# JuliaRobotics/IncrementalInference.jl

Hardware: AMD Instinct MI355X
Metric: clique-messages/sec (higher is better)
Workload: dtype f64; 1 GPU; config 2: ContinuousEuclid(2) 1000-variable odometry chain + priors every 100, N=200 particles, nested-dissection order, full up+down solveTree; variables_per_gpu=1000, particles=200, cliques=983, parallelism=single GPU

## Files before the change

### include/nbp.h

```cpp
#ifndef NBP_H
#define NBP_H

#include <stdint.h>

#ifdef __cplusplus
extern "C" {
#endif

#define NBP_MAXV 6
#define NBP_MAXF 128
#define NBP_MAXD 3
#define NBP_MAXC 4
#define NBP_MAXK 8
#define NBP_MAXN 512
#define NBP_COMP_STRIDE 13
enum nbp_dist {
  NBP_DIST_GAUSSIAN = 0,
  NBP_DIST_UNIFORM = 1,
  NBP_DIST_RAYLEIGH = 2,
  NBP_DIST_TABLE = 3
};

typedef int32_t nbp_status;
#define NBP_OK 0
// ... 65 lines not shown
typedef struct nbp_diag {
  int64_t solves;
  int64_t nonconverged;
  int64_t nan_results;
  int64_t residual_evals;
  int64_t lcv_evals;
  int64_t lcv_evals_f32;
  int64_t proposal_launches_workgroup;
  int64_t proposal_launches_wave;
  int64_t proposal_launches_split;
  int64_t lane_side_launches;
  int64_t lane_waits;
  int64_t lane_side_updates;
  int64_t sunk_updates;
  int64_t sink_launches;
} nbp_diag;

typedef struct nbp_ctx nbp_ctx;

int64_t nbp_arena_bytes(int32_t N, int32_t n_slots);
int64_t nbp_slot_stride_doubles(int32_t N);
nbp_status nbp_ctx_create(int32_t device, int32_t N, int32_t n_slots, void *arena,
                          int64_t arena_bytes, int32_t side_ints, nbp_ctx **out);
nbp_status nbp_ctx_destroy(nbp_ctx *ctx);
nbp_status nbp_ctx_attach(nbp_ctx *ctx, void *obj, void (*destroy)(void *obj));
void *nbp_ctx_attached(const nbp_ctx *ctx);
const char *nbp_last_error(void);
nbp_status nbp_synchronize(nbp_ctx *ctx);
void *nbp_arena_ptr(nbp_ctx *ctx);
void *nbp_stream_ptr(nbp_ctx *ctx);
// ... 278 lines not shown
nbp_status nbp_program_finalize(nbp_program *prog);
nbp_status nbp_program_run(nbp_program *prog, int32_t first_stage, int32_t last_stage );
nbp_status nbp_program_reseed(nbp_program *prog, uint64_t salt);
nbp_status nbp_program_num_seeds(nbp_program *prog, int32_t *out);
nbp_status nbp_program_set_seeds(nbp_program *prog, const uint64_t *seeds, int32_t n);
nbp_status nbp_program_seed_order(nbp_program *prog, int32_t *order, int32_t n);
nbp_status nbp_program_num_stages(nbp_program *prog, int32_t *out);
nbp_status nbp_program_num_fused(nbp_program *prog, int32_t *out);
nbp_status nbp_program_num_two_stream(nbp_program *prog, int32_t *out);
nbp_status nbp_program_set_lanes(nbp_program *prog, int32_t stage, const int32_t *lane_of_descriptor, int32_t n);
typedef struct nbp_lane_part_rec {
  int32_t stage, lane, first_desc, n, wait, signals;
} nbp_lane_part_rec;
nbp_status nbp_program_lane_plan(nbp_program *prog, nbp_lane_part_rec *out, int32_t cap, int32_t *n_out);
nbp_status nbp_program_sink_plan(nbp_program *prog, int32_t *gained, int32_t cap, int32_t *n_out);
nbp_status nbp_program_destroy(nbp_program *prog);
nbp_status nbp_program_retire(nbp_program *prog);

#define NBP_COMM_ID_BYTES 128
typedef struct nbp_comm nbp_comm;
#ifndef NBP_XFER_DEFINED
#define NBP_XFER_DEFINED
typedef struct nbp_xfer { int32_t peer; int32_t slot; } nbp_xfer;
#endif
nbp_status nbp_comm_unique_id(void *id_out );
nbp_status nbp_comm_create(nbp_ctx *ctx, int32_t world, int32_t rank, const void *id, nbp_comm **out);
nbp_status nbp_comm_destroy(nbp_comm *comm);
nbp_status nbp_comm_info(nbp_comm *comm, int32_t *nranks_out, int32_t *rank_out);
nbp_status nbp_exchange(nbp_ctx *ctx, nbp_comm *comm, const nbp_xfer *sends, int32_t n_sends, const nbp_xfer *recvs, int32_t n_recvs);

// ... 68 lines not shown
```

### incrementalinference.jl_amd/abi.py

```python
import ctypes as C
import os

MAXV, MAXF, MAXD, MAXC, MAXN, COMP_STRIDE = 6, 128, 3, 4, 512, 13

EUCLID1, EUCLID2, EUCLID3, CIRCULAR, SE2 = 1, 2, 3, 4, 5
F_PRIOR, F_MSGPRIOR, F_LINREL, F_CIRCULAR, F_SE2, F_EUCLIDDIST, F_PASSTHROUGH = 1, 2, 3, 4, 5, 6, 7
DIST_GAUSSIAN, DIST_UNIFORM, DIST_RAYLEIGH, DIST_TABLE = 0, 1, 2, 3
STAGE_PROPOSALS, STAGE_PRODUCTS, STAGE_COPIES, STAGE_DECONV, STAGE_COPY_POINTS = 1, 2, 3, 4, 5
OPT_LAZY_BANDWIDTH = 1
OPT_GRAPH_REPLAY = 2
OPT_FUSED_UPDATES = 3
OPT_ASYNC_UPLOAD = 4
OPT_UP_PASS_SINKS = 5

MANIFOLD_DIM = {EUCLID1: 1, EUCLID2: 2, EUCLID3: 3, CIRCULAR: 1, SE2: 3}
MANIFOLD_P = {EUCLID1: 1, EUCLID2: 2, EUCLID3: 3, CIRCULAR: 1, SE2: 6}


class ProposalDesc(C.Structure):
    _fields_ = [
        ("factor_kind", C.c_int32),
        ("manifold", C.c_int32),
        ("nvars", C.c_int32),
        ("sfidx", C.c_int32),
# ... 152 lines not shown
    _fields_ = [
        ("solves", C.c_int64),
        ("nonconverged", C.c_int64),
        ("nan_results", C.c_int64),
        ("residual_evals", C.c_int64),
        ("lcv_evals", C.c_int64),
        ("lcv_evals_f32", C.c_int64),
        ("proposal_launches_workgroup", C.c_int64),
        ("proposal_launches_wave", C.c_int64),
        ("proposal_launches_split", C.c_int64),
        ("lane_side_launches", C.c_int64),
        ("lane_waits", C.c_int64),
        ("lane_side_updates", C.c_int64),
        ("sunk_updates", C.c_int64),
        ("sink_launches", C.c_int64),
    ]


class LanePartRec(C.Structure):
    _fields_ = [("stage", C.c_int32), ("lane", C.c_int32), ("first_desc", C.c_int32), ("n", C.c_int32), ("wait", C.c_int32), ("signals", C.c_int32)]


class ProductPlanReq(C.Structure):
    _fields_ = [(k, C.c_int32) for k in ("N", "n", "F", "D", "mani", "geom_n")]


PLAN_REFUSED_BIG_IN_ROUND, PLAN_REFUSED_LDS, PLAN_REFUSED_NO_KERNEL = 1, 2, 3


class _PlanRec(C.Structure):
    def as_dict(self):
        return {k: (getattr(self, k).decode() if k == "kernel" else getattr(self, k)) for k, _ in self._fields_ if not k.startswith("pad")}


class ProductPlanRec(_PlanRec):
# ... 46 lines not shown
def slot_stride(N):
    return 3 * N + 8


_PKG_DIR = os.path.dirname(os.path.abspath(__file__))
LIB_PATH = os.path.join(_PKG_DIR, "csrc", "libnbp.so")

EXPORTS = [
    "nbp_arena_bytes", "nbp_slot_stride_doubles", "nbp_ctx_create", "nbp_ctx_destroy",
    "nbp_last_error", "nbp_synchronize", "nbp_arena_ptr", "nbp_stream_ptr", "nbp_ctx_particles", "nbp_ctx_slots", "nbp_ctx_device",
    "nbp_ctx_reserve_resident", "nbp_ctx_resident", "nbp_belief_write_batch_async", "nbp_belief_read_batch_begin", "nbp_belief_read_batch_end",
    "nbp_run_copies_async", "nbp_program_retire",
    "nbp_slot_write", "nbp_slot_read", "nbp_belief_write", "nbp_belief_read", "nbp_belief_write_batch", "nbp_belief_read_batch", "nbp_run_resample", "nbp_side_write", "nbp_side_read",
    "nbp_run_proposals", "nbp_run_bandwidth", "nbp_run_ppe", "nbp_kde_ppe", "nbp_run_evaluate", "nbp_kde_evaluate", "nbp_run_marginal_grid", "nbp_kde_marginal_grid", "nbp_run_evaluate_marginal", "nbp_run_mmd", "nbp_kde_mmd", "nbp_run_meancov", "nbp_kde_meancov", "nbp_run_kld", "nbp_kde_kld", "nbp_run_overlap", "nbp_kde_overlap", "nbp_run_overlap_search", "nbp_run_scene_grid", "nbp_run_credible", "nbp_kde_credible", "nbp_run_modes", "nbp_kde_modes", "nbp_run_mixture", "nbp_kde_mixture", "nbp_run_factor_likelihood", "nbp_factor_likelihood", "nbp_run_factor_mode_likelihood", "nbp_factor_mode_likelihood", "nbp_run_product_grid", "nbp_product_grid", "nbp_heatmap_create", "nbp_heatmap_build", "nbp_heatmap_draw", "nbp_heatmap_info", "nbp_heatmap_destroy", "nbp_heatmap_scan_eval", "nbp_heatmap_search_eval", "nbp_run_products", "nbp_run_copies", "nbp_run_deconv", "nbp_kde_bandwidth", "nbp_conv", "nbp_manifold_product",
    "nbp_program_create", "nbp_program_add_stage", "nbp_program_set_option", "nbp_program_finalize", "nbp_program_run",
    "nbp_program_reseed", "nbp_program_num_seeds", "nbp_program_set_seeds", "nbp_program_seed_order", "nbp_ctx_attach", "nbp_ctx_attached", "nbp_program_num_stages", "nbp_program_num_fused", "nbp_program_num_two_stream", "nbp_program_set_lanes", "nbp_program_lane_plan", "nbp_program_sink_plan", "nbp_program_destroy",
    "nbp_timing_enable", "nbp_timing_read", "nbp_timing_read_n", "nbp_diag_read",
    "nbp_plan_products", "nbp_plan_fits", "nbp_plan_proposals", "nbp_last_plans",
    "nbp_comm_unique_id", "nbp_comm_create", "nbp_comm_destroy", "nbp_comm_info", "nbp_exchange", "nbp_math_eval",
]

_lib = None


def load_library(path=None):
    global _lib
    if _lib is not None and path is None:
        return _lib
    path = path or os.environ.get("NBP_LIB_OVERRIDE") or LIB_PATH
    if not os.path.exists(path):
        raise RuntimeError(
# ... 92 lines not shown
    lib.nbp_program_destroy.argtypes = [vp]
    lib.nbp_comm_unique_id.argtypes = [vp]
    lib.nbp_comm_create.argtypes = [vp, i32, i32, vp, C.POINTER(vp)]
    lib.nbp_comm_destroy.argtypes = [vp]
    lib.nbp_comm_info.argtypes = [vp, ip, ip]
    lib.nbp_math_eval.argtypes = [vp, i32, dp, dp, dp, dp, i64]
    lib.nbp_exchange.argtypes = [vp, vp, C.POINTER(Xfer), i32, C.POINTER(Xfer), i32]
    lib.nbp_timing_enable.argtypes = [vp, i32]
    lib.nbp_timing_read.argtypes = [vp, dp, C.POINTER(i64)]
    lib.nbp_timing_read_n.argtypes = [vp, dp, C.POINTER(i64), i32]
    lib.nbp_program_num_fused.argtypes = [vp, C.POINTER(i32)]
    lib.nbp_program_num_two_stream.argtypes = [vp, C.POINTER(i32)]
    lib.nbp_program_set_lanes.argtypes = [vp, i32, ip, i32]
    lib.nbp_program_lane_plan.argtypes = [vp, C.POINTER(LanePartRec), i32, C.POINTER(i32)]
    lib.nbp_program_sink_plan.argtypes = [vp, C.POINTER(i32), i32, C.POINTER(i32)]
    lib.nbp_diag_read.argtypes = [vp, C.POINTER(Diag), i32]
    lib.nbp_plan_products.argtypes = [C.POINTER(ProductPlanReq), C.POINTER(ProductPlanRec), i64]
    lib.nbp_plan_fits.argtypes = [C.POINTER(FitPlanReq), C.POINTER(FitPlanRec), i64]
    lib.nbp_plan_proposals.argtypes = [C.POINTER(ProposalPlanReq), C.POINTER(ProposalPlanRec), i64]
    lib.nbp_last_plans.argtypes = [vp, C.POINTER(ProductPlanRec), C.POINTER(FitPlanRec), C.POINTER(FitPlanRec)]
    for name in EXPORTS:
        fn = getattr(lib, name)
        if fn.restype is C.c_int:
            fn.restype = C.c_int32
    if path == LIB_PATH:
        _lib = lib
    return lib
```

### incrementalinference.jl_amd/backend.py

```python
import ctypes as C
import weakref

import numpy as np

from . import abi


class NbpError(RuntimeError):
    """Hard error from libnbp (status < 0).  The Julia shim maps this to `error()`, which fails
    the clique Task and makes `monitorCSMs` tear the solve down with a CompositeException
    (reference: CliqStateMachineUtils.jl:184-246, test/testCSMMonitor.jl:51)."""


_IP, _DP = C.POINTER(C.c_int32), C.POINTER(C.c_double)


def _i32(seq):
    a = np.ascontiguousarray(seq, dtype=np.int32)
    return a, a.ctypes.data_as(_IP)


def _f64(a, shape=None):
    a = np.ascontiguousarray(a, dtype=np.float64)
    a = a if shape is None else a.reshape(shape)
# ... 712 lines not shown

    def lane_plan(self):
        n = C.c_int32(0)
        self.backend._check(self.backend.lib.nbp_program_lane_plan(self._p, None, 0, C.byref(n)))
        recs = (abi.LanePartRec * max(n.value, 1))()
        self.backend._check(self.backend.lib.nbp_program_lane_plan(self._p, recs, n.value, C.byref(n)))
        return [{k: getattr(r, k) for k, _ in abi.LanePartRec._fields_} for r in recs[:n.value]]

    def sink_plan(self):
        n = C.c_int32(0)
        self.backend._check(self.backend.lib.nbp_program_sink_plan(self._p, None, 0, C.byref(n)))
        arr = (C.c_int32 * max(n.value, 1))()
        self.backend._check(self.backend.lib.nbp_program_sink_plan(self._p, arr, n.value, C.byref(n)))
        return list(arr[:n.value])

    def num_fused(self):
        n = C.c_int32(0)
        self.backend._check(self.backend.lib.nbp_program_num_fused(self._p, C.byref(n)))
        return n.value

    def num_two_stream(self):
        n = C.c_int32(0)
        self.backend._check(self.backend.lib.nbp_program_num_two_stream(self._p, C.byref(n)))
        return n.value

    def run(self, first=0, last=-1):
        self.backend._check(self.backend.lib.nbp_program_run(self._p, first, last))

    def reseed(self, salt):
        self.backend._check(self.backend.lib.nbp_program_reseed(self._p, C.c_uint64(salt)))
# ... 40 lines not shown
```

### incrementalinference.jl_amd/csrc/nbp_api.hip

```cpp
#include <hip/hip_runtime.h>

#include <cmath>
#include <cstdio>
#include <cstring>
#include <string>
#include <thread>
#include <vector>

#include <unordered_map>

#include <dlfcn.h>
#include <algorithm>
#include <rccl/rccl.h>

#ifndef NBP_TU
#define NBP_TU 0
#endif
#include "nbp_kernels.h"
#include "nbp_fused.h"
#include "nbp_ppe.h"
#include "nbp_query.h"
#include "nbp_stats.h"
#include "nbp_marginal.h"
#include "nbp_heatmap.h"
#include "nbp_modes.h"
#include "nbp_likelihood.h"
#include "nbp_overlap.h"
#include "nbp_credible.h"
#include "nbp_mixture.h"
#include "nbp_scene.h"
#include "nbp_productgrid.h"
#include "../../include/nbp_lanes.h"
#include "../../include/nbp_sinks.h"

static thread_local std::string g_err;
static nbp_status fail(nbp_status code, const std::string &msg) {
  g_err = msg;
  return code;
}
template <class F>
static void host_parallel_for(int n, int grain, F &&f) {
  const unsigned hw = std::thread::hardware_concurrency();
  int nt = n / grain;
  if (nt > 8) nt = 8;
  if (hw && nt > (int)hw) nt = (int)hw;
  if (nt <= 1) {
    for (int i = 0; i < n; i++) f(i);
    return;
// ... 65 lines not shown
  int prop_split_min = -1;
  int64_t prop_launches[3] = {0, 0, 0};
  int fused_p1_min = 2048;
  hipStream_t stream2 = nullptr;
  hipEvent_t pipe_ev[2] = {nullptr, nullptr};
  int pipe_min = 1 << 30;
  bool no_lanes = false;
  std::vector<hipEvent_t> lane_ev;
  hipEvent_t lane_fork = nullptr, lane_join = nullptr;
  double *gstats1 = nullptr;
  size_t gstats1_doubles = 0;
  int64_t lane_side_launches = 0, lane_waits = 0, lane_side_updates = 0;
  bool no_sinks = false;
  int sink_placement = 0;
  int64_t sunk_updates = 0, sink_launches = 0;
  int lcv_p2_min = 256, lcv_p1_min = 4 * 256;
  bool fit_w5 = true, debug_occupancy = false;
  int prod_hl2_min = 192, prod_nch = 0, prod_all_levels_hl = 8;
  bool prod_xs = true, prod_lat_uni = true;
  nbp_product_plan_rec last_product{};
  nbp_fit_plan_rec last_prep{}, last_fit{};
  bool timing = false;
  std::vector<std::pair<hipEvent_t, hipEvent_t>> ev[5];
  double ms[5] = {0, 0, 0, 0, 0};
  int64_t nl[5] = {0, 0, 0, 0, 0};
};

typedef void (*nbp_product_fn)(const nbp_product_desc *, double *, const double *, int, double *, int, int64_t, int32_t *, nbp_levels);
struct nbp_product_kernel_row { nbp_product_fn fn; int HL, mani; bool xs, w1; const char *name; int lb; };
#define NBP_ROW(NAME, HL_, MANI_, XS_, W1_, LB_) {NAME, HL_, MANI_, XS_, W1_, #NAME, LB_}
// ... 141 lines not shown
  c->S = nbp_slot_stride_doubles(N);
  c->Npad = ((N + 63) / 64) * 64;
  c->P = 1024 / c->Npad;
  if (c->P > 4) c->P = 4;
  if (c->P < 1) c->P = 1;
  c->threads = c->P * c->Npad;
  c->spec_on = getenv("NBP_NO_SPECULATIVE_FITS") == nullptr;
  c->spec_depth3 = !(getenv("NBP_SPEC_DEPTH3") && atoi(getenv("NBP_SPEC_DEPTH3")) == 0);
  c->fused_on = getenv("NBP_NO_FUSED_UPDATE") == nullptr;
  if (getenv("NBP_FUSED_MIN")) c->fused_min = atoi(getenv("NBP_FUSED_MIN"));
  if (getenv("NBP_PROPOSAL_WAVE_MIN")) c->prop_wave_min = atoi(getenv("NBP_PROPOSAL_WAVE_MIN"));
  if (getenv("NBP_PROPOSAL_SPLIT_MIN")) c->prop_split_min = atoi(getenv("NBP_PROPOSAL_SPLIT_MIN"));
  if (getenv("NBP_PIPELINE_MIN")) c->pipe_min = atoi(getenv("NBP_PIPELINE_MIN"));
  c->no_lanes = getenv("NBP_NO_LANES") && atoi(getenv("NBP_NO_LANES")) != 0;
  c->no_sinks = getenv("NBP_NO_SINKS") && atoi(getenv("NBP_NO_SINKS")) != 0;
  if (getenv("NBP_SINK_PLACEMENT")) c->sink_placement = atoi(getenv("NBP_SINK_PLACEMENT"));
  if (getenv("NBP_FUSED_P1_MIN")) c->fused_p1_min = atoi(getenv("NBP_FUSED_P1_MIN"));
  if (getenv("NBP_PRODUCT_HL2_MIN")) c->prod_hl2_min = atoi(getenv("NBP_PRODUCT_HL2_MIN"));
  if (getenv("NBP_PRODUCT_NCH")) c->prod_nch = atoi(getenv("NBP_PRODUCT_NCH"));
  if (getenv("NBP_PRODUCT_ALL_LEVELS_HL")) c->prod_all_levels_hl = atoi(getenv("NBP_PRODUCT_ALL_LEVELS_HL"));
  c->prod_xs = getenv("NBP_NO_XS_PRODUCTS") == nullptr;
  c->prod_lat_uni = getenv("NBP_NO_UNIFORM_LATENCY_PRODUCTS") == nullptr;
  if (getenv("NBP_LCV_P2_MIN")) c->lcv_p2_min = atoi(getenv("NBP_LCV_P2_MIN"));
  if (getenv("NBP_LCV_P1_MIN")) c->lcv_p1_min = atoi(getenv("NBP_LCV_P1_MIN"));
  c->fit_w5 = getenv("NBP_NO_W5_FITS") == nullptr;
  c->debug_occupancy = getenv("NBP_DEBUG_OCCUPANCY") != nullptr;
}

nbp_status nbp_ctx_create(int32_t device, int32_t N, int32_t n_slots, void *arena, int64_t arena_bytes,
                          int32_t side_ints, nbp_ctx **out) {
// ... 710 lines not shown
  const int nblocks = env.geom_blocks ? env.geom_blocks : 2 * nbw + 2 * nprod;
  f.P = c->P;
  if (nblocks > c->lcv_p2_min && f.P > 2) f.P = 2;
  if (nblocks > c->lcv_p1_min) f.P = 1;
  if (c->spec_on && nbw > 0 && nbw <= NBP_SPEC_MAXJOBS && !env.geom_n) {
    if (c->spec_depth3 && coords * 7 + nkd <= NBP_SPEC_MAXBLOCKS) f.depth = 3;
    else if (coords * 3 + nkd <= NBP_SPEC_MAXBLOCKS) f.depth = 2;
  }
  f.KS = f.depth ? (1 << f.depth) - 1 : 1;
  f.w5 = !f.depth && c->fit_w5 && f.P == 1 && ((c->Npad >> 6) & 3) == 1 && c->Npad > 64;
  f.threads = f.P * c->Npad;
  if (nbw > 0) f.lds = nbp_bandwidth_lds_bytes(c->N, c->Npad, f.P);
  if (nkd > 0) f.lds = std::max(f.lds, nbp_kd_lds_bytes(3, c->N, c->Npad, f.P));
  return f;
}
static nbp_fit_plan_rec fit_plan_rec(const nbp_ctx *c, const nbp_launch_env &env, int nbw, int coords, int nprod, int kdF, bool prep, const nbp_fit_plan &f) {
  nbp_fit_plan_rec r{};
  r.status = NBP_OK;
  r.P = f.P; r.depth = f.depth; r.KS = f.KS; r.w5 = f.w5; r.threads = f.threads; r.prep = prep;
  r.N = c->N; r.fits = nbw; r.coords = coords; r.products = nprod; r.kdF = kdF; r.geom_blocks = env.geom_blocks;
  r.lds = (int64_t)f.lds;
  snprintf(r.kernel, sizeof(r.kernel), "%s%s", prep ? "nbp_prep_kernel" : "nbp_bandwidth_kernel", f.depth == 3 ? "_spec<3>" : (f.depth == 2 ? "_spec<2>" : (f.w5 ? "_w5" : "")));
  return r;
}

static const int NBP_PRODUCT_LAT_WAVES = 4;
static const int NBP_PRODUCT_THR_WAVES = 8;
static const int NBP_PRODUCT_CIRC_WAVES = 4;
static const int NBP_PRODUCT_WIDE_WAVES = 16;
static const size_t NBP_PRODUCT_LDS_CAP = 150 * 1024;
// ... 1681 lines not shown
  size_t upd_off = 0;
  nbp_fits split_out;
  bool pipe = false;
  int pipe_split = -1, pipe_ent = 0;
  std::vector<int> moved_to;
  std::vector<int32_t> lane_hint;
  int lane_split = -1;
  std::vector<int> sink_to;
  int sink_stay = -1;
  size_t gather_off = 0;
  int gather_n = 0, gained = 0;
  std::vector<std::pair<int, int>> gather_src;
  bool sink_touched = false, gathered = false;
  int lane = 0, user = -1;
  nbp_fits bound;
  std::vector<int> waits;
  bool signals = false;
};
struct nbp_program {
  nbp_ctx *ctx = nullptr;
  std::vector<nbp_stage> stages;
  std::vector<char> blob;
  char *dev = nullptr;
  size_t dev_bytes = 0;
  bool finalized = false;
  bool lazy_bw = false;
  bool use_graph = true;
  bool use_fused = true;
  bool async_upload = false;
  int n_user_stages = 0;
// ... 578 lines not shown
        for (const auto &src : st.gather_src) g.push_back(dead_row(src.first)[(size_t)src.second]);
        dead.push_back(g.data());
      } else {
        dead.push_back(row.empty() ? nullptr : row.data() + from);
      }
      parts.push_back(std::move(pt));
    }
  }
  p->first_part[(size_t)p->n_user_stages] = (int)parts.size();
  {
    nbp_stage pt;
    pt.user = p->n_user_stages;
    dead.push_back(nullptr);
    parts.push_back(std::move(pt));
  }
  nbp_fits pend[2];
  std::vector<nbp_fits> ran(parts.size());
  for (int k = 0; k < (int)parts.size(); k++) {
    nbp_stage &st = parts[(size_t)k];
    const int l = st.lane, o = 1 - l;
    const char *d = p->blob.data() + st.offset;
    if (k == p->first_part[(size_t)st.user]) {
      st.bound = pend[0];
      for (const nbp_fits::fit &f : pend[1].v) st.bound.push(f.slot, f.mani);
    }
    if (st.kind == NBP_STAGE_DECONV || st.kind == NBP_STAGE_COPY_POINTS)
      stage_writes(p, st, [&](int, int32_t slot) { pend[0].drop(slot); pend[1].drop(slot); });
    if (!pend[o].empty()) {
      auto claim = [&](int32_t slot) {
        for (size_t i = 0; i < pend[o].v.size();)
          if (pend[o].v[i].slot == slot) { pend[l].v.push_back(pend[o].v[i]); pend[o].v.erase(pend[o].v.begin() + (long)i); } else i++;
      };
      stage_reads(p, st, [&](int, int32_t slot, nbp_access a) { if (a != NBP_RD_POINTS || st.kind == NBP_STAGE_PRODUCTS) claim(slot); });
      if (st.kind == NBP_STAGE_PROPOSALS || st.kind == NBP_STAGE_PRODUCTS) stage_writes(p, st, [&](int, int32_t slot) { claim(slot); });
      if (st.kind == NBP_STAGE_COPIES || st.kind == 0) {
        for (const nbp_fits::fit &f : pend[o].v) pend[l].v.push_back(f);
        pend[o].clear();
      }
    }
    st.ent = pend[l];
    auto flush_if_read = [&](nbp_access what) {
      stage_reads(p, st, [&](int, int32_t slot, nbp_access a) { st.flush_before |= a == what && pend[l].has(slot); });
      if (st.flush_before) { for (const nbp_fits::fit &f : pend[l].v) ran[(size_t)k].push(f.slot, f.mani); pend[l].clear(); }
    };
    if (st.kind == NBP_STAGE_PROPOSALS) {
      flush_if_read(NBP_RD_KDE);
      queue_fits(pend[l], (const nbp_proposal_desc *)d, st.n, dead[(size_t)k]);
    } else if (st.kind == NBP_STAGE_PRODUCTS) {
      const nbp_product_desc *qd = (const nbp_product_desc *)d;
      st.need_prep = false;
      for (int i = 0; i < st.n; i++) st.need_prep |= qd[i].nfactors > 1;
      flush_if_read(NBP_RD_POINTS);
      if (st.need_prep) {
        for (const nbp_fits::fit &f : pend[l].v) ran[(size_t)k].push(f.slot, f.mani);
        pend[l].clear();
      } else {
        for (int i = 0; i < st.n; i++) pend[l].rename(qd[i].in_slot[0], qd[i].out_slot);
        pend[l].dedup();
      }
      queue_fits(pend[l], qd, st.n, dead[(size_t)k]);
    } else if (st.kind == NBP_STAGE_DECONV || st.kind == NBP_STAGE_COPY_POINTS) {
      if (st.kind == NBP_STAGE_DECONV)
        for (int i = 0; i < st.n; i++) pend[l].push(((const nbp_proposal_desc *)d)[i].out_slot, ((const nbp_proposal_desc *)d)[i].manifold);
    } else {
      st.flush_before = true;
      for (const nbp_fits::fit &f : pend[l].v) ran[(size_t)k].push(f.slot, f.mani);
      pend[l].clear();
    }
  }
  std::vector<nbp_lane_part> sw(parts.size());
  for (int k = 0; k < (int)parts.size(); k++) {
    const nbp_stage &st = parts[(size_t)k];
    nbp_lane_part &a = sw[(size_t)k];
    a.stage = st.user;
    a.lane = st.lane;
    a.barrier = st.kind == 0 || ((st.kind == NBP_STAGE_COPIES || st.kind == NBP_STAGE_COPY_POINTS) && st.n == 0);
    stage_touches(p, st, [&](int, int32_t x) { a.reads.push_back(x); }, [&](int, int32_t x) { a.writes.push_back(x); });
    for (const nbp_fits::fit &f : ran[(size_t)k].v) { a.reads.push_back(2 * f.slot); a.writes.push_back(2 * f.slot + 1); }
  }
  nbp_lane_sweep(sw);
  for (int k = 0; k < (int)parts.size(); k++) {
    parts[(size_t)k].waits = sw[(size_t)k].waits;
    parts[(size_t)k].signals = sw[(size_t)k].signals;
  }
  for (const nbp_stage &st : parts)
    if (st.lane == 1 && st.kind == NBP_STAGE_PRODUCTS && st.n > 0) {
      p->lane_ws = std::max(p->lane_ws, (size_t)st.n * (size_t)(st.maxfd / 4) * nbp_kd_ws_doubles(p->ctx->N));
      nbp_launch_env env = ctx_env(p->ctx);
      p->lane_gstats = std::max(p->lane_gstats, std::max(product_plan(p->ctx, env, st.n, st.maxfd, st.mani).gstats, product_plan(p->ctx, env, st.n, st.maxfd, -1).gstats));
    }
}

static void layout_blob(nbp_program *p) {
  for (nbp_stage &st : p->stages) append_fits(p->blob, st.ent);
  for (nbp_stage &st : p->stages)
    if (st.fused_second) append_fits(p->blob, st.split_out, 4);
  for (nbp_stage &st : p->parts) {
    append_fits(p->blob, st.ent);
    append_fits(p->blob, st.bound);
  }
  for (nbp_stage &st : p->stages)
    if (st.fused) {
      st.upd_off = (p->blob.size() + 63) & ~(size_t)63;
      p->blob.resize(st.upd_off + st.upd.size() * sizeof(nbp_update_desc));
      memcpy(p->blob.data() + st.upd_off, st.upd.data(), st.upd.size() * sizeof(nbp_update_desc));
    }
  std::vector<int64_t> so;
  for (int s = 0; s < p->n_user_stages; s++) {
    const nbp_stage &st = p->stages[s];
    if (st.kind == NBP_STAGE_PROPOSALS || st.kind == NBP_STAGE_DECONV)
      for (int i = 0; i < st.n; i++) {
        const size_t o = st.offset + (size_t)(st.moved_to.empty() ? i : st.moved_to[(size_t)i]) * sizeof(nbp_proposal_desc);
        so.push_back((int64_t)(o + offsetof(nbp_proposal_desc, seed)));
// ... 194 lines not shown
    seek(0);
    seek(1);
    if (nx[0] >= k1 && nx[1] >= k1) break;
    const int l = nx[1] < k1 && (ready(nx[1]) || nx[0] >= k1) ? 1 : 0;
    const int k = nx[l]++;
    issued[(size_t)(k - k0)] = 1;
    const nbp_stage &st = p->parts[(size_t)k];
    nbp_launch_env &e = env[st.lane];
    for (int w : st.waits)
      if (w >= k0) {
        LANECHK(hipStreamWaitEvent(e.stream, ev[(size_t)(w - k0)], 0));
        c->lane_waits++;
      }
    int launches = 0;
    nbp_status rc = NBP_OK;
    if (st.flush_before && st.ent.size()) { rc = launch_bandwidth(c, e, fits_dev(st.ent, p->dev)); launches++; }
    if (rc) return rc;
    if (st.kind == NBP_STAGE_PROPOSALS) {
      rc = launch_proposals(c, e, (const nbp_proposal_desc *)(p->dev + st.offset), st.n, st.mani);
      launches += st.n > 0;
    } else if (st.kind == NBP_STAGE_PRODUCTS) {
      const nbp_product_desc *dd = (const nbp_product_desc *)(p->dev + st.offset);
      if (st.need_prep) { rc = launch_prep(c, e, fits_dev(st.ent, p->dev), dd, st.n, st.maxfd, st.mani); launches++; }
      if (!rc) rc = launch_products(c, e, dd, st.n, st.maxfd, st.mani);
      launches += st.n > 0;
      if (st.lane) c->lane_side_updates += st.n;
    } else if (st.kind == NBP_STAGE_DECONV) {
      rc = launch_deconv(c, (const nbp_proposal_desc *)(p->dev + st.offset), nullptr, st.n);
    } else {
      rc = launch_copies(c, (const nbp_copy_desc *)(p->dev + st.offset), st.n, st.kind == NBP_STAGE_COPY_POINTS, e.stream);
      launches += st.n > 0;
    }
    if (rc) return rc;
    if (st.lane) c->lane_side_launches += launches;
    if (st.gained) {
      c->sink_launches += launches;
      if (st.kind == NBP_STAGE_PRODUCTS) c->sunk_updates += st.gained;
    }
    if (st.signals) {
      if (nev >= c->lane_ev.size()) return fail(NBP_ERR_RANGE, "lanes: fewer events than signalling parts (sized at nbp_program_finalize)");
      ev[(size_t)(k - k0)] = c->lane_ev[nev++];
      LANECHK(hipEventRecord(ev[(size_t)(k - k0)], e.stream));
    }
  }
  LANECHK(hipEventRecord(c->lane_join, c->stream2));
  LANECHK(hipStreamWaitEvent(c->stream, c->lane_join, 0));
#undef LANECHK
  return launch_bandwidth(c, ctx_env(c), fits_dev(p->parts[(size_t)k1].bound, p->dev));
}

static nbp_status run_range(nbp_program *p, int first, int last) {
  if (lanes_apply(p, first, last)) return run_lanes(p, first, last);
  nbp_ctx *c = p->ctx;
  nbp_launch_env env = ctx_env(c);
  for (int s = first; s < last; s++) {
    const nbp_stage &st = p->stages[s];
    nbp_status rc = NBP_OK;
    if (st.flush_before) rc = launch_bandwidth(c, env, fits_dev(st.ent, p->dev));
    if (rc) return rc;
    if (st.kind == NBP_STAGE_PROPOSALS && st.fused && s + 1 >= last) {
      rc = launch_proposals(c, env, (const nbp_proposal_desc *)(p->dev + st.offset), st.n, st.mani);
    } else if (st.kind == NBP_STAGE_PROPOSALS && st.fused) {
// ... 178 lines not shown
                       sizeof(nbp_copy_desc) : sizeof(nbp_proposal_desc));
    out[k] = {st.user, st.lane, st.gathered ? 0 : (int32_t)((st.offset - us.offset) / esz), st.n, st.waits.empty() ? -1 : st.waits[0], st.signals ? 1 : 0};
  }
  return NBP_OK;
}

nbp_status nbp_program_sink_plan(nbp_program *p, int32_t *gained, int32_t cap, int32_t *n_out) {
  if (!p || !n_out || (!gained && cap > 0)) return fail(NBP_ERR_ARG, "null argument");
  if (!p->finalized) return fail(NBP_ERR_ARG, "program not finalized");
  const int np = p->parts.empty() ? 0 : (int)p->parts.size() - 1;
  *n_out = np;
  for (int k = 0; k < np && k < cap; k++) gained[k] = p->parts[(size_t)k].gained;
  return NBP_OK;
}

static void program_free(nbp_program *p, bool sync);
static void reap_retired(nbp_ctx *c) {
  for (size_t i = 0; i < c->retired.size();) {
    if (hipEventQuery(c->retired[i].second) == hipSuccess) {
      hipEventDestroy(c->retired[i].second);
      nbp_program *p = c->retired[i].first;
      c->retired.erase(c->retired.begin() + (long)i);
      program_free(p, false);
    } else
      i++;
  }
}
nbp_status nbp_program_retire(nbp_program *p) {
  if (!p) return NBP_OK;
  if (!p->ctx) { delete p; return NBP_OK; }
// ... 331 lines not shown
  out->nonconverged = (int64_t)h.nonconverged;
  out->nan_results = (int64_t)h.nan_results;
  out->residual_evals = (int64_t)h.residual_evals;
  out->lcv_evals = (int64_t)h.lcv_evals;
  out->lcv_evals_f32 = (int64_t)h.lcv_evals_f32;
  out->proposal_launches_workgroup = c->prop_launches[0];
  out->proposal_launches_wave = c->prop_launches[1];
  out->proposal_launches_split = c->prop_launches[2];
  if (reset) c->prop_launches[0] = c->prop_launches[1] = c->prop_launches[2] = 0;
  out->lane_side_launches = c->lane_side_launches;
  out->lane_waits = c->lane_waits;
  out->lane_side_updates = c->lane_side_updates;
  if (reset) c->lane_side_launches = c->lane_waits = c->lane_side_updates = 0;
  out->sunk_updates = c->sunk_updates;
  out->sink_launches = c->sink_launches;
  if (reset) c->sunk_updates = c->sink_launches = 0;
  if (reset) HIPCHK(hipMemset(c->counters, 0, offsetof(nbp_counters, flags)));
  return NBP_OK;
}

#ifdef NBP_PHASE_TIMING
nbp_status nbp_debug_phase_read(long long *out, int n, int reset) {
  long long h[64];
  HIPCHK(hipDeviceSynchronize());
  HIPCHK(hipMemcpyFromSymbol(h, HIP_SYMBOL(nbp_phase_clk), sizeof(h)));
  for (int i = 0; i < n && i < 64; i++) out[i] = h[i];
  if (reset) {
    memset(h, 0, sizeof(h));
    HIPCHK(hipMemcpyToSymbol(HIP_SYMBOL(nbp_phase_clk), h, sizeof(h)));
  }
  return NBP_OK;
// ... 19 lines not shown
```

Measured before the change: 156,600 messages/s.

## Factor fit scheduling into a placement walk that can defer bandwidth fits

Moves the logic that decides where pending KDE bandwidth fits are flushed into a standalone walk over program parts. An optional placement mode can hold a fit until the next part that actually reads it, with a rule based on launch width, instead of flushing at stage order. Adds a diagnostic counter and a plan query API. The default mode stays stage order, so the default schedule should match the old behavior while the code path itself is rewritten.

```diff
diff --git a/include/nbp.h b/include/nbp.h
--- a/include/nbp.h
+++ b/include/nbp.h
@@ -103,6 +103,7 @@
   int64_t lane_side_updates;
   int64_t sunk_updates;
   int64_t sink_launches;
+  int64_t fits_placed_late;
 } nbp_diag;
 
 typedef struct nbp_ctx nbp_ctx;
@@ -411,6 +412,10 @@
 } nbp_lane_part_rec;
 nbp_status nbp_program_lane_plan(nbp_program *prog, nbp_lane_part_rec *out, int32_t cap, int32_t *n_out);
 nbp_status nbp_program_sink_plan(nbp_program *prog, int32_t *gained, int32_t cap, int32_t *n_out);
+typedef struct nbp_fit_part_rec {
+  int32_t stage, lane, pending, flush, prep, late, wide, flush_spec, prep_spec;
+} nbp_fit_part_rec;
+nbp_status nbp_program_fit_plan(nbp_program *prog, nbp_fit_part_rec *out, int32_t cap, int32_t *n_out);
 nbp_status nbp_program_destroy(nbp_program *prog);
 nbp_status nbp_program_retire(nbp_program *prog);
 
diff --git a/include/nbp_fits.h b/include/nbp_fits.h
--- /dev/null
+++ b/include/nbp_fits.h
@@ -0,0 +1,155 @@
+#ifndef NBP_FITS_H
+#define NBP_FITS_H
+#include <algorithm>
+#include <cstddef>
+#include <cstdint>
+#include <unordered_map>
+#include <utility>
+#include <vector>
+
+enum { NBP_FIT_STAGE_ORDER = 0, NBP_FIT_PLACE = 1, NBP_FIT_PLACE_STRICT = 2 };
+enum { NBP_FITP_ALL = 0, NBP_FITP_PROPOSALS = 1, NBP_FITP_PRODUCTS = 2, NBP_FITP_POINTS = 3 };
+
+struct nbp_fit { int32_t slot, mani; };
+
+struct nbp_fit_part {
+  int lane = 0;
+  int kind = NBP_FITP_ALL;
+  bool first_of_stage = false;
+  std::vector<int32_t> reads;
+  std::vector<int32_t> topup;
+  std::vector<int32_t> writes;
+  std::vector<int32_t> claims;
+  std::vector<std::pair<int32_t, int32_t>> carries;
+  std::vector<nbp_fit> queues;
+  bool prep = false;
+  bool wide = false;
+  std::vector<nbp_fit> ent;
+  std::vector<nbp_fit> flush;
+  std::vector<nbp_fit> prep_fits;
+  std::vector<nbp_fit> bound;
+  int pending = 0;
+  int late = 0;
+  int held = 0;
+};
+
+static inline void nbp_fit_walk(std::vector<nbp_fit_part> &parts, int mode) {
+  const bool place = mode != NBP_FIT_STAGE_ORDER;
+  const int np = (int)parts.size();
+  struct access { int part, how; };
+  std::unordered_map<int32_t, std::vector<access>> touch;
+  std::vector<int> next_all((size_t)np + 1, np);
+  for (int k = np - 1; k >= 0 && place; k--) next_all[(size_t)k] = parts[(size_t)k].kind == NBP_FITP_ALL ? k : next_all[(size_t)k + 1];
+  for (int k = 0; k < np && place; k++) {
+    const nbp_fit_part &a = parts[(size_t)k];
+    for (int32_t s : a.reads) touch[s].push_back({k, 0});
+    for (int32_t s : a.topup) touch[s].push_back({k, 1});
+    for (int32_t s : a.writes) touch[s].push_back({k, 2});
+  }
+  auto next_access = [&](int32_t slot, int k) -> access {
+    access r{next_all[(size_t)k + 1], 2};
+    auto it = touch.find(slot);
+    if (it == touch.end()) return r;
+    for (const access &t : it->second)
+      if (t.part > k) return t.part < r.part ? t : r;
+    return r;
+  };
+  auto has = [](const std::vector<nbp_fit> &v, int32_t slot) {
+    return std::any_of(v.begin(), v.end(), [&](const nbp_fit &f) { return f.slot == slot; });
+  };
+  auto drop = [](std::vector<nbp_fit> &v, int32_t slot) {
+    v.erase(std::remove_if(v.begin(), v.end(), [&](const nbp_fit &f) { return f.slot == slot; }), v.end());
+  };
+  std::vector<nbp_fit> pend[2];
+  struct held_fit { nbp_fit f; int lane; };
+  std::unordered_map<int32_t, std::vector<held_fit>> held;
+  auto held_sorted = [&]() {
+    std::vector<nbp_fit> hb;
+    for (const auto &h : held)
+      for (const held_fit &x : h.second) hb.push_back(x.f);
+    std::sort(hb.begin(), hb.end(), [](const nbp_fit &x, const nbp_fit &y) { return x.slot < y.slot; });
+    return hb;
+  };
+  for (int k = 0; k < np; k++) {
+    nbp_fit_part &a = parts[(size_t)k];
+    const int l = a.lane ? 1 : 0, o = 1 - l;
+    a.ent.clear(); a.flush.clear(); a.prep_fits.clear(); a.bound.clear();
+    a.pending = a.late = a.held = 0;
+    if (a.first_of_stage) {
+      a.bound = pend[0];
+      a.bound.insert(a.bound.end(), pend[1].begin(), pend[1].end());
+      const std::vector<nbp_fit> hb = held_sorted();
+      a.bound.insert(a.bound.end(), hb.begin(), hb.end());
+    }
+    if (a.kind == NBP_FITP_POINTS)
+      for (int32_t s : a.writes) { drop(pend[0], s); drop(pend[1], s); }
+    if (!pend[o].empty()) {
+      for (int32_t s : a.claims)
+        for (size_t i = 0; i < pend[o].size();)
+          if (pend[o][i].slot == s) { pend[l].push_back(pend[o][i]); pend[o].erase(pend[o].begin() + (long)i); } else i++;
+      if (a.kind == NBP_FITP_ALL) {
+        pend[l].insert(pend[l].end(), pend[o].begin(), pend[o].end());
+        pend[o].clear();
+      }
+    }
+    a.ent = pend[l];
+    a.pending = (int)pend[l].size();
+    for (const auto &h : held)
+      for (const held_fit &x : h.second) a.pending += x.lane == l;
+    if (!held.empty()) {
+      auto due = [&](int32_t s, bool to_prep) {
+        auto it = held.find(s);
+        if (it == held.end()) return;
+        for (const held_fit &x : it->second) { (to_prep ? a.prep_fits : a.flush).push_back(x.f); a.late++; }
+        held.erase(it);
+      };
+      if (a.kind == NBP_FITP_ALL) {
+        for (const nbp_fit &f : held_sorted()) due(f.slot, false);
+      } else {
+        const bool in_prep = a.kind == NBP_FITP_PRODUCTS && a.prep;
+        for (int32_t s : a.topup) due(s, false);
+        for (int32_t s : a.reads) due(s, in_prep);
+        for (int32_t s : a.writes) due(s, in_prep);
+      }
+    }
+    std::vector<nbp_fit> run;
+    bool all = false, twice = false;
+    if (a.kind == NBP_FITP_PROPOSALS) {
+      bool rd = false;
+      for (int32_t s : a.reads) rd = rd || has(pend[l], s);
+      if (rd) { run.swap(pend[l]); }
+    } else if (a.kind == NBP_FITP_PRODUCTS) {
+      bool top = false;
+      for (int32_t s : a.topup) top = top || has(pend[l], s);
+      if (top) { all = true; twice = a.prep; run.swap(pend[l]); }
+      else if (a.prep) { run.swap(pend[l]); }
+      if (!a.prep) {
+        for (const auto &c : a.carries)
+          for (nbp_fit &f : pend[l]) if (f.slot == c.first) f.slot = c.second;
+        for (size_t q = 0; q < pend[l].size(); q++)
+          pend[l].erase(std::remove_if(pend[l].begin() + (long)q + 1, pend[l].end(), [&](const nbp_fit &f) { return f.slot == pend[l][q].slot; }), pend[l].end());
+      }
+    } else if (a.kind == NBP_FITP_ALL) {
+      all = true;
+      run.swap(pend[l]);
+    }
+    const bool to_prep = a.kind == NBP_FITP_PRODUCTS && a.prep && !all;
+    for (const nbp_fit &f : run) {
+      bool here = all || !place;
+      if (!here) here = std::find(a.reads.begin(), a.reads.end(), f.slot) != a.reads.end() || std::find(a.writes.begin(), a.writes.end(), f.slot) != a.writes.end();
+      if (!here) {
+        const access t = next_access(f.slot, k);
+        const nbp_fit_part *b = t.part < np && t.how == 0 ? &parts[(size_t)t.part] : nullptr;
+        const bool wide_prep = b && b->kind == NBP_FITP_PRODUCTS && b->prep && b->wide;
+        if (a.wide) here = !(wide_prep && b->lane == a.lane);
+        else if (mode == NBP_FIT_PLACE_STRICT) here = false;
+        else here = !(wide_prep || (b && b->kind == NBP_FITP_PROPOSALS && b->wide));
+      }
+      if (!here) { held[f.slot].push_back({f, l}); a.held++; continue; }
+      (to_prep ? a.prep_fits : a.flush).push_back(f);
+      if (twice) a.prep_fits.push_back(f);
+    }
+    pend[l].insert(pend[l].end(), a.queues.begin(), a.queues.end());
+  }
+}
+#endif
diff --git a/incrementalinference.jl_amd/abi.py b/incrementalinference.jl_amd/abi.py
--- a/incrementalinference.jl_amd/abi.py
+++ b/incrementalinference.jl_amd/abi.py
@@ -190,11 +190,16 @@
         ("lane_side_updates", C.c_int64),
         ("sunk_updates", C.c_int64),
         ("sink_launches", C.c_int64),
+        ("fits_placed_late", C.c_int64),
     ]
 
 
 class LanePartRec(C.Structure):
     _fields_ = [("stage", C.c_int32), ("lane", C.c_int32), ("first_desc", C.c_int32), ("n", C.c_int32), ("wait", C.c_int32), ("signals", C.c_int32)]
+
+
+class FitPartRec(C.Structure):
+    _fields_ = [(k, C.c_int32) for k in ("stage", "lane", "pending", "flush", "prep", "late", "wide", "flush_spec", "prep_spec")]
 
 
 class ProductPlanReq(C.Structure):
@@ -271,7 +276,7 @@
     "nbp_slot_write", "nbp_slot_read", "nbp_belief_write", "nbp_belief_read", "nbp_belief_write_batch", "nbp_belief_read_batch", "nbp_run_resample", "nbp_side_write", "nbp_side_read",
     "nbp_run_proposals", "nbp_run_bandwidth", "nbp_run_ppe", "nbp_kde_ppe", "nbp_run_evaluate", "nbp_kde_evaluate", "nbp_run_marginal_grid", "nbp_kde_marginal_grid", "nbp_run_evaluate_marginal", "nbp_run_mmd", "nbp_kde_mmd", "nbp_run_meancov", "nbp_kde_meancov", "nbp_run_kld", "nbp_kde_kld", "nbp_run_overlap", "nbp_kde_overlap", "nbp_run_overlap_search", "nbp_run_scene_grid", "nbp_run_credible", "nbp_kde_credible", "nbp_run_modes", "nbp_kde_modes", "nbp_run_mixture", "nbp_kde_mixture", "nbp_run_factor_likelihood", "nbp_factor_likelihood", "nbp_run_factor_mode_likelihood", "nbp_factor_mode_likelihood", "nbp_run_product_grid", "nbp_product_grid", "nbp_heatmap_create", "nbp_heatmap_build", "nbp_heatmap_draw", "nbp_heatmap_info", "nbp_heatmap_destroy", "nbp_heatmap_scan_eval", "nbp_heatmap_search_eval", "nbp_run_products", "nbp_run_copies", "nbp_run_deconv", "nbp_kde_bandwidth", "nbp_conv", "nbp_manifold_product",
     "nbp_program_create", "nbp_program_add_stage", "nbp_program_set_option", "nbp_program_finalize", "nbp_program_run",
-    "nbp_program_reseed", "nbp_program_num_seeds", "nbp_program_set_seeds", "nbp_program_seed_order", "nbp_ctx_attach", "nbp_ctx_attached", "nbp_program_num_stages", "nbp_program_num_fused", "nbp_program_num_two_stream", "nbp_program_set_lanes", "nbp_program_lane_plan", "nbp_program_sink_plan", "nbp_program_destroy",
+    "nbp_program_reseed", "nbp_program_num_seeds", "nbp_program_set_seeds", "nbp_program_seed_order", "nbp_ctx_attach", "nbp_ctx_attached", "nbp_program_num_stages", "nbp_program_num_fused", "nbp_program_num_two_stream", "nbp_program_set_lanes", "nbp_program_lane_plan", "nbp_program_sink_plan", "nbp_program_fit_plan", "nbp_program_destroy",
     "nbp_timing_enable", "nbp_timing_read", "nbp_timing_read_n", "nbp_diag_read",
     "nbp_plan_products", "nbp_plan_fits", "nbp_plan_proposals", "nbp_last_plans",
     "nbp_comm_unique_id", "nbp_comm_create", "nbp_comm_destroy", "nbp_comm_info", "nbp_exchange", "nbp_math_eval",
@@ -394,6 +399,7 @@
     lib.nbp_program_set_lanes.argtypes = [vp, i32, ip, i32]
     lib.nbp_program_lane_plan.argtypes = [vp, C.POINTER(LanePartRec), i32, C.POINTER(i32)]
     lib.nbp_program_sink_plan.argtypes = [vp, C.POINTER(i32), i32, C.POINTER(i32)]
+    lib.nbp_program_fit_plan.argtypes = [vp, C.POINTER(FitPartRec), i32, C.POINTER(i32)]
     lib.nbp_diag_read.argtypes = [vp, C.POINTER(Diag), i32]
     lib.nbp_plan_products.argtypes = [C.POINTER(ProductPlanReq), C.POINTER(ProductPlanRec), i64]
     lib.nbp_plan_fits.argtypes = [C.POINTER(FitPlanReq), C.POINTER(FitPlanRec), i64]
diff --git a/incrementalinference.jl_amd/backend.py b/incrementalinference.jl_amd/backend.py
--- a/incrementalinference.jl_amd/backend.py
+++ b/incrementalinference.jl_amd/backend.py
@@ -750,6 +750,13 @@
         self.backend._check(self.backend.lib.nbp_program_sink_plan(self._p, arr, n.value, C.byref(n)))
         return list(arr[:n.value])
 
+    def fit_plan(self):
+        n = C.c_int32(0)
+        self.backend._check(self.backend.lib.nbp_program_fit_plan(self._p, None, 0, C.byref(n)))
+        recs = (abi.FitPartRec * max(n.value, 1))()
+        self.backend._check(self.backend.lib.nbp_program_fit_plan(self._p, recs, n.value, C.byref(n)))
+        return [{k: getattr(r, k) for k, _ in abi.FitPartRec._fields_} for r in recs[:n.value]]
+
     def num_fused(self):
         n = C.c_int32(0)
         self.backend._check(self.backend.lib.nbp_program_num_fused(self._p, C.byref(n)))
diff --git a/incrementalinference.jl_amd/csrc/nbp_api.hip b/incrementalinference.jl_amd/csrc/nbp_api.hip
--- a/incrementalinference.jl_amd/csrc/nbp_api.hip
+++ b/incrementalinference.jl_amd/csrc/nbp_api.hip
@@ -32,6 +32,7 @@
 #include "nbp_productgrid.h"
 #include "../../include/nbp_lanes.h"
 #include "../../include/nbp_sinks.h"
+#include "../../include/nbp_fits.h"
 
 static thread_local std::string g_err;
 static nbp_status fail(nbp_status code, const std::string &msg) {
@@ -127,6 +128,9 @@
   bool no_sinks = false;
   int sink_placement = 0;
   int64_t sunk_updates = 0, sink_launches = 0;
+  int fit_placement = NBP_FIT_STAGE_ORDER;
+  int fit_wide_min = -1;
+  int64_t fits_placed_late = 0;
   int lcv_p2_min = 256, lcv_p1_min = 4 * 256;
   bool fit_w5 = true, debug_occupancy = false;
   int prod_hl2_min = 192, prod_nch = 0, prod_all_levels_hl = 8;
@@ -298,6 +302,9 @@
   if (getenv("NBP_PIPELINE_MIN")) c->pipe_min = atoi(getenv("NBP_PIPELINE_MIN"));
   c->no_lanes = getenv("NBP_NO_LANES") && atoi(getenv("NBP_NO_LANES")) != 0;
   c->no_sinks = getenv("NBP_NO_SINKS") && atoi(getenv("NBP_NO_SINKS")) != 0;
+  if (getenv("NBP_FIT_PLACEMENT")) c->fit_placement = atoi(getenv("NBP_FIT_PLACEMENT")) == 2 ? NBP_FIT_PLACE_STRICT : (atoi(getenv("NBP_FIT_PLACEMENT")) == 1 ? NBP_FIT_PLACE : NBP_FIT_STAGE_ORDER);
+  if (getenv("NBP_NO_FIT_PLACEMENT") && atoi(getenv("NBP_NO_FIT_PLACEMENT")) != 0) c->fit_placement = NBP_FIT_STAGE_ORDER;
+  if (getenv("NBP_FIT_WIDE_MIN")) c->fit_wide_min = atoi(getenv("NBP_FIT_WIDE_MIN"));
   if (getenv("NBP_SINK_PLACEMENT")) c->sink_placement = atoi(getenv("NBP_SINK_PLACEMENT"));
   if (getenv("NBP_FUSED_P1_MIN")) c->fused_p1_min = atoi(getenv("NBP_FUSED_P1_MIN"));
   if (getenv("NBP_PRODUCT_HL2_MIN")) c->prod_hl2_min = atoi(getenv("NBP_PRODUCT_HL2_MIN"));
@@ -1038,6 +1045,9 @@
   if (nkd > 0) f.lds = std::max(f.lds, nbp_kd_lds_bytes(3, c->N, c->Npad, f.P));
   return f;
 }
+static bool fit_launch_wide(const nbp_ctx *c, int nreads, int nprod) {
+  return 2 * nreads + 2 * nprod > (c->fit_wide_min >= 0 ? c->fit_wide_min : c->lcv_p1_min);
+}
 static nbp_fit_plan_rec fit_plan_rec(const nbp_ctx *c, const nbp_launch_env &env, int nbw, int coords, int nprod, int kdF, bool prep, const nbp_fit_plan &f) {
   nbp_fit_plan_rec r{};
   r.status = NBP_OK;
@@ -2749,6 +2759,9 @@
   bool sink_touched = false, gathered = false;
   int lane = 0, user = -1;
   nbp_fits bound;
+  nbp_fits flush, prep_fits;
+  int fits_pending = 0, fits_late = 0;
+  bool fit_wide = false;
   std::vector<int> waits;
   bool signals = false;
 };
@@ -3357,59 +3370,55 @@
     dead.push_back(nullptr);
     parts.push_back(std::move(pt));
   }
-  nbp_fits pend[2];
-  std::vector<nbp_fits> ran(parts.size());
+  std::vector<nbp_fit_part> fp(parts.size());
   for (int k = 0; k < (int)parts.size(); k++) {
     nbp_stage &st = parts[(size_t)k];
-    const int l = st.lane, o = 1 - l;
+    nbp_fit_part &a = fp[(size_t)k];
     const char *d = p->blob.data() + st.offset;
-    if (k == p->first_part[(size_t)st.user]) {
-      st.bound = pend[0];
-      for (const nbp_fits::fit &f : pend[1].v) st.bound.push(f.slot, f.mani);
-    }
-    if (st.kind == NBP_STAGE_DECONV || st.kind == NBP_STAGE_COPY_POINTS)
-      stage_writes(p, st, [&](int, int32_t slot) { pend[0].drop(slot); pend[1].drop(slot); });
-    if (!pend[o].empty()) {
-      auto claim = [&](int32_t slot) {
-        for (size_t i = 0; i < pend[o].v.size();)
-          if (pend[o].v[i].slot == slot) { pend[l].v.push_back(pend[o].v[i]); pend[o].v.erase(pend[o].v.begin() + (long)i); } else i++;
-      };
-      stage_reads(p, st, [&](int, int32_t slot, nbp_access a) { if (a != NBP_RD_POINTS || st.kind == NBP_STAGE_PRODUCTS) claim(slot); });
-      if (st.kind == NBP_STAGE_PROPOSALS || st.kind == NBP_STAGE_PRODUCTS) stage_writes(p, st, [&](int, int32_t slot) { claim(slot); });
-      if (st.kind == NBP_STAGE_COPIES || st.kind == 0) {
-        for (const nbp_fits::fit &f : pend[o].v) pend[l].v.push_back(f);
-        pend[o].clear();
-      }
-    }
-    st.ent = pend[l];
-    auto flush_if_read = [&](nbp_access what) {
-      stage_reads(p, st, [&](int, int32_t slot, nbp_access a) { st.flush_before |= a == what && pend[l].has(slot); });
-      if (st.flush_before) { for (const nbp_fits::fit &f : pend[l].v) ran[(size_t)k].push(f.slot, f.mani); pend[l].clear(); }
-    };
+    a.lane = st.lane;
+    a.first_of_stage = k == p->first_part[(size_t)st.user];
+    a.kind = st.kind == NBP_STAGE_PROPOSALS ? NBP_FITP_PROPOSALS : (st.kind == NBP_STAGE_PRODUCTS ? NBP_FITP_PRODUCTS :
+             (st.kind == NBP_STAGE_DECONV || st.kind == NBP_STAGE_COPY_POINTS ? NBP_FITP_POINTS : NBP_FITP_ALL));
+    stage_reads(p, st, [&](int, int32_t slot, nbp_access acc) {
+      if (acc != NBP_RD_POINTS) a.reads.push_back(slot);
+      else if (st.kind == NBP_STAGE_PRODUCTS) a.topup.push_back(slot);
+      if (acc != NBP_RD_POINTS || st.kind == NBP_STAGE_PRODUCTS) a.claims.push_back(slot);
+    });
+    if (a.kind == NBP_FITP_ALL) continue;
+    stage_writes(p, st, [&](int, int32_t slot) {
+      a.writes.push_back(slot);
+      if (a.kind != NBP_FITP_POINTS) a.claims.push_back(slot);
+    });
+    nbp_fits q;
     if (st.kind == NBP_STAGE_PROPOSALS) {
-      flush_if_read(NBP_RD_KDE);
-      queue_fits(pend[l], (const nbp_proposal_desc *)d, st.n, dead[(size_t)k]);
+      queue_fits(q, (const nbp_proposal_desc *)d, st.n, dead[(size_t)k]);
     } else if (st.kind == NBP_STAGE_PRODUCTS) {
       const nbp_product_desc *qd = (const nbp_product_desc *)d;
       st.need_prep = false;
       for (int i = 0; i < st.n; i++) st.need_prep |= qd[i].nfactors > 1;
-      flush_if_read(NBP_RD_POINTS);
-      if (st.need_prep) {
-        for (const nbp_fits::fit &f : pend[l].v) ran[(size_t)k].push(f.slot, f.mani);
-        pend[l].clear();
-      } else {
-        for (int i = 0; i < st.n; i++) pend[l].rename(qd[i].in_slot[0], qd[i].out_slot);
-        pend[l].dedup();
-      }
-      queue_fits(pend[l], qd, st.n, dead[(size_t)k]);
-    } else if (st.kind == NBP_STAGE_DECONV || st.kind == NBP_STAGE_COPY_POINTS) {
-      if (st.kind == NBP_STAGE_DECONV)
-        for (int i = 0; i < st.n; i++) pend[l].push(((const nbp_proposal_desc *)d)[i].out_slot, ((const nbp_proposal_desc *)d)[i].manifold);
-    } else {
-      st.flush_before = true;
-      for (const nbp_fits::fit &f : pend[l].v) ran[(size_t)k].push(f.slot, f.mani);
-      pend[l].clear();
-    }
+      a.prep = st.need_prep;
+      for (int i = 0; i < st.n && !st.need_prep; i++) a.carries.push_back({qd[i].in_slot[0], qd[i].out_slot});
+      queue_fits(q, qd, st.n, dead[(size_t)k]);
+    } else if (st.kind == NBP_STAGE_DECONV) {
+      for (int i = 0; i < st.n; i++) q.push(((const nbp_proposal_desc *)d)[i].out_slot, ((const nbp_proposal_desc *)d)[i].manifold);
+    }
+    for (const nbp_fits::fit &f : q.v) a.queues.push_back({f.slot, f.mani});
+    std::vector<int32_t> distinct(a.reads);
+    std::sort(distinct.begin(), distinct.end());
+    a.wide = fit_launch_wide(p->ctx, (int)(std::unique(distinct.begin(), distinct.end()) - distinct.begin()), a.prep ? st.n : 0);
+  }
+  nbp_fit_walk(fp, p->ctx->fit_placement);
+  std::vector<nbp_fits> ran(parts.size());
+  for (int k = 0; k < (int)parts.size(); k++) {
+    nbp_stage &st = parts[(size_t)k];
+    const nbp_fit_part &a = fp[(size_t)k];
+    for (const nbp_fit &f : a.bound) st.bound.push(f.slot, f.mani);
+    for (const nbp_fit &f : a.flush) { st.flush.push(f.slot, f.mani); ran[(size_t)k].push(f.slot, f.mani); }
+    for (const nbp_fit &f : a.prep_fits) { st.prep_fits.push(f.slot, f.mani); ran[(size_t)k].push(f.slot, f.mani); }
+    st.flush_before = !st.flush.empty();
+    st.fits_pending = a.pending;
+    st.fits_late = a.late;
+    st.fit_wide = a.wide;
   }
   std::vector<nbp_lane_part> sw(parts.size());
   for (int k = 0; k < (int)parts.size(); k++) {
@@ -3439,7 +3448,8 @@
   for (nbp_stage &st : p->stages)
     if (st.fused_second) append_fits(p->blob, st.split_out, 4);
   for (nbp_stage &st : p->parts) {
-    append_fits(p->blob, st.ent);
+    append_fits(p->blob, st.flush);
+    append_fits(p->blob, st.prep_fits);
     append_fits(p->blob, st.bound);
   }
   for (nbp_stage &st : p->stages)
@@ -3664,14 +3674,15 @@
       }
     int launches = 0;
     nbp_status rc = NBP_OK;
-    if (st.flush_before && st.ent.size()) { rc = launch_bandwidth(c, e, fits_dev(st.ent, p->dev)); launches++; }
+    if (st.flush.size()) { rc = launch_bandwidth(c, e, fits_dev(st.flush, p->dev)); launches++; }
     if (rc) return rc;
+    c->fits_placed_late += st.fits_late;
     if (st.kind == NBP_STAGE_PROPOSALS) {
       rc = launch_proposals(c, e, (const nbp_proposal_desc *)(p->dev + st.offset), st.n, st.mani);
       launches += st.n > 0;
     } else if (st.kind == NBP_STAGE_PRODUCTS) {
       const nbp_product_desc *dd = (const nbp_product_desc *)(p->dev + st.offset);
-      if (st.need_prep) { rc = launch_prep(c, e, fits_dev(st.ent, p->dev), dd, st.n, st.maxfd, st.mani); launches++; }
+      if (st.need_prep) { rc = launch_prep(c, e, fits_dev(st.prep_fits, p->dev), dd, st.n, st.maxfd, st.mani); launches++; }
       if (!rc) rc = launch_products(c, e, dd, st.n, st.maxfd, st.mani);
       launches += st.n > 0;
       if (st.lane) c->lane_side_updates += st.n;
@@ -3696,6 +3707,7 @@
   LANECHK(hipEventRecord(c->lane_join, c->stream2));
   LANECHK(hipStreamWaitEvent(c->stream, c->lane_join, 0));
 #undef LANECHK
+  if (p->parts[(size_t)k1].kind == 0) c->fits_placed_late += p->parts[(size_t)k1].fits_late;
   return launch_bandwidth(c, ctx_env(c), fits_dev(p->parts[(size_t)k1].bound, p->dev));
 }
 
@@ -3904,6 +3916,28 @@
   return NBP_OK;
 }
 
+nbp_status nbp_program_fit_plan(nbp_program *p, nbp_fit_part_rec *out, int32_t cap, int32_t *n_out) {
+  if (!p || !n_out || (!out && cap > 0)) return fail(NBP_ERR_ARG, "null argument");
+  PROG_ALIVE(p);
+  if (!p->finalized) return fail(NBP_ERR_ARG, "program not finalized");
+  const int np = p->parts.empty() ? 0 : (int)p->parts.size();
+  *n_out = np;
+  const nbp_launch_env env = ctx_env(p->ctx);
+  auto geometry = [](const nbp_fit_plan &f) { return f.depth == 3 ? 3 : (f.depth == 2 ? 2 : 0); };
+  for (int k = 0; k < np && k < cap; k++) {
+    const nbp_stage &st = p->parts[(size_t)k];
+    const bool prep = st.kind == NBP_STAGE_PRODUCTS && st.need_prep;
+    const nbp_fits &fl = st.kind == 0 ? st.bound : st.flush;
+    nbp_fit_part_rec r{};
+    r.stage = st.user; r.lane = st.lane; r.pending = st.fits_pending; r.flush = fl.size(); r.prep = prep ? st.prep_fits.size() : -1;
+    r.late = st.fits_late; r.wide = st.fit_wide ? 1 : 0;
+    r.flush_spec = fl.size() ? geometry(fit_plan(p->ctx, env, fl.size(), fl.coords())) : -1;
+    r.prep_spec = prep ? geometry(fit_plan(p->ctx, env, st.prep_fits.size(), st.prep_fits.coords(), st.n, st.maxfd / 4)) : -1;
+    out[k] = r;
+  }
+  return NBP_OK;
+}
+
 static void program_free(nbp_program *p, bool sync);
 static void reap_retired(nbp_ctx *c) {
   for (size_t i = 0; i < c->retired.size();) {
@@ -4265,7 +4299,8 @@
   if (reset) c->lane_side_launches = c->lane_waits = c->lane_side_updates = 0;
   out->sunk_updates = c->sunk_updates;
   out->sink_launches = c->sink_launches;
-  if (reset) c->sunk_updates = c->sink_launches = 0;
+  out->fits_placed_late = c->fits_placed_late;
+  if (reset) c->sunk_updates = c->sink_launches = c->fits_placed_late = 0;
   if (reset) HIPCHK(hipMemset(c->counters, 0, offsetof(nbp_counters, flags)));
   return NBP_OK;
 }
```

New measurement: 156,200 messages/s. Within noise of the previous version (-0.3%).
